# abb128/april-asr

Measured on AMD Instinct MI355X. Metric: audio_seconds_per_second (concurrent 16 kHz sessions x 1/RTF), aprilv0_en-us-sized streaming RNN-T, higher is better.
Workload: dtype f32

## Files before the change

april_asr_amd/csrc/kernels_gemm_kw.hip:

```cpp
#include "kernels.h"
#include "device_utils.h"
#include <algorithm>
#include <atomic>
#include <cstdio>
#include <cstdlib>

namespace aprilx {

namespace {

template <class T> __device__ __forceinline__ T gload(const void *p) { return *(const __attribute__((address_space(1))) T *)(p); }
template <class T> __device__ __forceinline__ void gstore(void *p, const T &v) { *(__attribute__((address_space(1))) T *)(p) = v; }

template <int N> __device__ __forceinline__ void wait_vm()
{
    __builtin_amdgcn_s_waitcnt(0x0F70 | (N & 15) | ((N >> 4) << 14));
}
__device__ __forceinline__ void wait_lgkm0() { __builtin_amdgcn_s_waitcnt(0xC07F); }

constexpr int NW = 8, D = 2;
template <int MT, int NT> struct KwGeom {
    static constexpr int BM = 16 * MT, BN = 16 * NT, LDR = BN + 4, NTH = 64 * NW;
    static constexpr int STAGE_BYTES = BM * 128;
    static constexpr int RING_BYTES = D * STAGE_BYTES, PLANE_BYTES = BM * LDR * 4;
    static constexpr int WAVE_BYTES = ((RING_BYTES > PLANE_BYTES ? RING_BYTES : PLANE_BYTES) + 1023) / 1024 * 1024;
    static constexpr int LDS_MAIN = NW * WAVE_BYTES;
    static constexpr int PLANE = WAVE_BYTES / 4;
    static constexpr int NPIECE = 2 * MT;
    static constexpr int LX = NPIECE, LY = 2 * NT, GSZ = LX + LY;
};

template <int MT, int NT, int EPI, int CPW>
__device__ __forceinline__ void gemm_kw_body(const GemmArgs &g, const int bx, const int by, const unsigned wg_linear)
{
    using G = KwGeom<MT, NT>;
    constexpr int BM = G::BM, BN = G::BN, LDR = G::LDR, NTH = G::NTH, PLANE = G::PLANE;
    constexpr bool ROW_EPI = EPI == EPI_HR || EPI == EPI_RESID_SSQ;
    static_assert(ROW_EPI, "no GM_KW form of this epilogue");
    static_assert(CPW == 1 || CPW == 4, "a wave owns one chunk or one slab");
    constexpr bool DB1 = MT * NT >= 16;
    extern __shared__ __attribute__((aligned(1024))) float red[];
    char *lds = reinterpret_cast<char *>(red);

    if (g.run_flag && gload<int>(g.run_flag) != g.run_gen) return;
    const int lane = threadIdx.x & 63;
    const int wave = __builtin_amdgcn_readfirstlane(threadIdx.x >> 6);
#ifdef APRIL_GEMM_TRACE
    auto stamp = [&](int i) { if (g.trace && wave == 0) g.trace[(size_t)wg_linear * 16 + i] = __builtin_amdgcn_s_memtime(); };
    unsigned long long ph_acc[5] = {0, 0, 0, 0, 0}, ph_t = 0;
    auto lap = [&](int i) { const unsigned long long now = __builtin_amdgcn_s_memtime(); ph_acc[i] += now - ph_t; ph_t = now; };
#else
    auto stamp = [](int) {};
    auto lap = [](int) {};
    (void)wg_linear;
#endif
    stamp(0);
    const int nt0 = bx * NT, n0 = bx * BN, m0 = by * BM;
    const int KB = g.K >> 4;
    const int c = KB / (4 * g.kz);
    constexpr int cpw = CPW;
    const int T = cpw * c;
// ... 30 lines not shown
        }
        if (aidx) {
#pragma unroll
            for (int i = 0; i < G::NPIECE; ++i) arows[i] = gload<int>(aidx + arows[i]);
        }
#pragma unroll
        for (int i = 0; i < G::NPIECE; ++i) {
            const int R = i * 8 + (lane >> 3);
            const int gseg = (lane & 7) ^ ((R >> 1) & 7);
            aoff[i] = (uint32_t)((size_t)arows[i] * lda * 4 + gseg * 16);
        }
    }
    char *my = lds + wave * G::WAVE_BYTES;
    auto issue_dma = [&](int slot) {
#ifdef APRIL_KW_ABLATE
        if (g.debug == 4 || g.debug == 6 || g.debug == 7 || g.debug == 9) return;
#endif
#pragma unroll
        for (int i = 0; i < G::NPIECE; ++i) {
            __builtin_amdgcn_global_load_lds((const __attribute__((address_space(1))) void *)(abase + aoff[i]),
                                             (__attribute__((address_space(3))) void *)(my + slot * G::STAGE_BYTES + i * 1024), 16, 0, 0);
        }
#ifdef APRIL_KW_ABLATE
        if (g.debug == 3) return;
#endif
        abase += 128;
    };
    const char *bp = reinterpret_cast<const char *>(g.wp) + ((size_t)nt0 * KB + first_kb) * 1024;
    const size_t bstride = (size_t)KB * 1024;
    const uint32_t boff = (uint32_t)lane * 16u;
    constexpr int DB = DB1 ? 1 : D;
    f32x4 be[DB][NT], bo[DB][NT];
#ifdef APRIL_KW_ABLATE
#pragma unroll
    for (int t = 0; t < DB; ++t)
#pragma unroll
        for (int nt = 0; nt < NT; ++nt) { be[t][nt] = f32x4{1.f, 1.f, 1.f, 1.f}; bo[t][nt] = be[t][nt]; }
#endif
    auto load_b = [&](f32x4 (&b)[NT]) {
#ifdef APRIL_KW_ABLATE
        if (g.debug == 6 || g.debug == 7 || g.debug == 8) {
#pragma unroll
            for (int nt = 0; nt < NT; ++nt) asm volatile("" : "+v"(b[nt]));
            return;
        }
#endif
#pragma unroll
        for (int nt = 0; nt < NT; ++nt) b[nt] = gload<f32x4>(bp + nt * bstride + boff);
#ifdef APRIL_KW_ABLATE
        if (g.debug == 3) return;
#endif
        bp += 1024;
    };

    constexpr int QROW = BN / 4, NQ = BM * QROW, QPT = (NQ + NTH - 1) / NTH;
    f32x4 e_bias[QPT], e_res[QPT];
// ... 9 lines not shown
        const int qn = q < NQ ? n0 + (q % QROW) * 4 : n0;
        e_bias[i] = (EPI != EPI_HR) ? gload<f32x4>(g.bias + qn) : f32x4{0.f, 0.f, 0.f, 0.f};
        e_slot[i] = (EPI == EPI_HR && g.slot_idx) ? gload<int>(g.slot_idx + m) : m;
        e_res[i] = (EPI == EPI_HR || (EPI == EPI_RESID_SSQ && g.resid)) ? gload<f32x4>(g.resid + (size_t)m * g.ldr + qn) : f32x4{0.f, 0.f, 0.f, 0.f};
    }
    };
    constexpr bool LATE_EPI = DB1 || (MT == 1 && EPI == EPI_HR);
    if constexpr (!LATE_EPI) fetch_epilogue_operands();

    const int mrow = lane & 15, kq = lane >> 4;
    int a_rd[2];
#pragma unroll
    for (int p = 0; p < 2; ++p) a_rd[p] = mrow * 128 + (((p * 4 + kq) ^ ((mrow >> 1) & 7)) << 4);
    auto read_frags = [&](int slot, int p, f32x4 (&a)[MT]) {
#ifdef APRIL_KW_ABLATE
        if (g.debug == 6) {
#pragma unroll
            for (int mt = 0; mt < MT; ++mt) asm volatile("" : "+v"(a[mt]));
            return;
        }
#endif
#pragma unroll
        for (int mt = 0; mt < MT; ++mt) a[mt] = *reinterpret_cast<const f32x4 *>(my + slot * G::STAGE_BYTES + a_rd[p] + mt * 2048);
    };

    f32x4 acc[MT][NT], S[CPW == 4 ? MT : 1][CPW == 4 ? NT : 1];
#define APRIL_KW_EACH(expr) _Pragma("unroll") for (int mt = 0; mt < MT; ++mt) _Pragma("unroll") for (int nt = 0; nt < NT; ++nt) { expr; }
    APRIL_KW_EACH(acc[mt][nt] = (f32x4{0.f, 0.f, 0.f, 0.f}))
    int chunk_i = 0, in_chunk = 0;
    auto fold = [&]() {
        if constexpr (CPW == 4) {
            const bool first = chunk_i == 0;
#pragma unroll
            for (int mt = 0; mt < MT; ++mt)
#pragma unroll
                for (int nt = 0; nt < NT; ++nt) {
                    S[mt][nt] = first ? acc[mt][nt] : S[mt][nt] + acc[mt][nt];
                    acc[mt][nt] = f32x4{0.f, 0.f, 0.f, 0.f};
                    if constexpr (MT * NT >= 16) __builtin_amdgcn_sched_barrier(0);
                }
            ++chunk_i;
        }
    };
    auto mfma_block = [&](const f32x4 (&a)[MT], const f32x4 (&b)[NT]) {
#ifdef APRIL_KW_ABLATE
// ... 45 lines not shown
                    __builtin_amdgcn_sched_barrier(0);
                }
                wait_lgkm0();
                if (more_a) issue_dma(slot);
                if (more_b) load_b(be[0]);
#pragma unroll
                for (int mt = 0; mt < MT; ++mt) {
                    mfma_mt(mt, bo[0]);
                    __builtin_amdgcn_sched_barrier(0);
                    if (mt == 0) { if (more_a) wait_vm<G::NPIECE + 3 * NT>(); else if (more_b) wait_vm<3 * NT>(); }
                    read_frag1(slot ^ 1, 0, mt);
                    __builtin_amdgcn_sched_barrier(0);
                }
                if (more_b) load_b(bo[0]);
                if constexpr (CPW == 4) { if (++in_chunk == cs) { in_chunk = 0; fold(); } }
            }
        }
    } else
    if (g.debug != 1) {
#pragma unroll
        for (int t = 0; t < D; ++t) { issue_dma(t); load_b(be[t]); load_b(bo[t]); }
        wait_vm<(D - 1) * G::GSZ + G::LY>();
        __builtin_amdgcn_sched_barrier(0);
        read_frags(0, 0, a0);
        stamp(1);
        auto stage = [&](const int slot, const bool more, auto wait_next) {
            read_frags(slot, 1, a1);
            __builtin_amdgcn_sched_barrier(0);
            mfma_block(a0, be[slot]);
            __builtin_amdgcn_sched_barrier(0);
// ... 80 lines not shown
        } else {
            const bool ok = e_ok[i];
            f32x4 y = f32x4{0.f, 0.f, 0.f, 0.f};
            if (ok) {
                y = resid_tail(v, e_bias[i], e_res[i], g.resid != nullptr);
                gstore<f32x4>(g.out + (size_t)m * g.ldo + n, y);
            }
            float ss;
            if (granule_ssq_store(y, ok, q, ss)) gstore<float>(g.ssq_out + (size_t)m * (g.N / SSQ_COLS) + n / SSQ_COLS, ss);
        }
    }
    stamp(4);
#undef APRIL_KW_EACH
}

template <int MT, int NT, int EPI, int CPW>
__global__ __launch_bounds__(64 * NW, (MT == 1 && EPI == EPI_HR) ? 6 : 2) void gemm_kw_kernel(GemmArgs g)
{
    gemm_kw_body<MT, NT, EPI, CPW>(g, (int)blockIdx.x, (int)blockIdx.y, blockIdx.x + gridDim.x * blockIdx.y);
}

template <int MT, int NT, int EPI, int CPW>
__global__ __launch_bounds__(64 * NW, (MT == 1 && EPI == EPI_HR) ? 6 : 2) void gemm_kw_zkernel(const GemmArgs *__restrict__ zargs)
{
    const GemmArgs g = zargs[blockIdx.z];
    gemm_kw_body<MT, NT, EPI, CPW>(g, (int)blockIdx.x, (int)blockIdx.y, blockIdx.x + gridDim.x * (blockIdx.y + gridDim.y * blockIdx.z));
}

template <int MT, int NT, int EPI, int CPW>
void launch_kw_one(const GemmArgs &g, const GemmArgs *dev_args, int n, hipStream_t s)
{
    using G = KwGeom<MT, NT>;
    dim3 grid((unsigned)(g.N / G::BN), (unsigned)((g.M + G::BM - 1) / G::BM), (unsigned)std::max(1, n));
    const size_t lds = (size_t)G::LDS_MAIN + scale_lds_floats(g, G::BM) * sizeof(float);
    launch_gemm_pair<&gemm_kw_kernel<MT, NT, EPI, CPW>, &gemm_kw_zkernel<MT, NT, EPI, CPW>>(grid, dim3(G::NTH), lds, true, s, g, dev_args);
}

template <int MT, int NT>
bool dispatch_kw(const GemmArgs &g, const GemmArgs *dev_args, int n, hipStream_t s)
{
    const int cpw = 4 * g.kz / NW;
    if (g.epi == EPI_HR && cpw == 4) { launch_kw_one<MT, NT, EPI_HR, 4>(g, dev_args, n, s); return true; }
    if (g.epi == EPI_HR && cpw == 1) { launch_kw_one<MT, NT, EPI_HR, 1>(g, dev_args, n, s); return true; }
    if (g.epi == EPI_RESID_SSQ && cpw == 4) { launch_kw_one<MT, NT, EPI_RESID_SSQ, 4>(g, dev_args, n, s); return true; }
    if (g.epi == EPI_RESID_SSQ && cpw == 1) { launch_kw_one<MT, NT, EPI_RESID_SSQ, 1>(g, dev_args, n, s); return true; }
    return false;
}

}

// ... 28 lines not shown
```

Measured before the change: 20490.

## Add hand-scheduled inline-asm main loop for split-K GEMM tiles

Replaces the compiler-generated K loop of the wave-split-K GEMM, for the NT=2, MT=1 or 2, four-chunks-per-wave forms, with a hand-written inline-assembly loop. The loop interleaves MFMA instructions with LDS DMA issues, B-operand global loads and LDS fragment reads, and uses explicit waitcnt values and an in-register chunk fold. The aim is tighter overlap of memory traffic with matrix math and fewer compiler-inserted stalls. In exchange it hardcodes register allocation and wait counts, adds a large fragile asm block, and can be turned off with an environment variable.

```diff
diff --git a/april_asr_amd/csrc/gemm_kw_asm.inc b/april_asr_amd/csrc/gemm_kw_asm.inc
--- /dev/null
+++ b/april_asr_amd/csrc/gemm_kw_asm.inc
@@ -0,0 +1,693 @@
+#define APRIL_KWLOOP_M2_TEXT \
+    "s_mov_b32 s90, m0\n" \
+    "s_mov_b64 s[80:81], %[ap]\n" \
+    "s_mov_b64 s[82:83], %[bp0]\n" \
+    "s_mov_b64 s[84:85], %[bp1]\n" \
+    "s_mov_b32 s89, %[lds]\n" \
+    "s_lshr_b32 s86, %[nst], 1\n" \
+    "s_sub_u32 s86, s86, 1\n" \
+    "s_mov_b32 s88, %[cs]\n" \
+    "s_mov_b32 s87, 0\n" \
+    "s_nop 4\n" \
+    "s_add_u32 m0, s89, 0\n" \
+    "s_nop 0\n" \
+    "global_load_lds_dwordx4 %[ao0], s[80:81]\n" \
+    "s_add_u32 m0, s89, 1024\n" \
+    "s_nop 0\n" \
+    "global_load_lds_dwordx4 %[ao1], s[80:81]\n" \
+    "s_add_u32 m0, s89, 2048\n" \
+    "s_nop 0\n" \
+    "global_load_lds_dwordx4 %[ao2], s[80:81]\n" \
+    "s_add_u32 m0, s89, 3072\n" \
+    "s_nop 0\n" \
+    "global_load_lds_dwordx4 %[ao3], s[80:81]\n" \
+    "s_add_u32 s80, s80, 128\n" \
+    "s_addc_u32 s81, s81, 0\n" \
+    "global_load_dwordx4 v[88:91], %[bo], s[82:83]\n" \
+    "global_load_dwordx4 v[92:95], %[bo], s[84:85]\n" \
+    "global_load_dwordx4 v[96:99], %[bo], s[82:83] offset:1024\n" \
+    "global_load_dwordx4 v[100:103], %[bo], s[84:85] offset:1024\n" \
+    "s_add_u32 s82, s82, 2048\n" \
+    "s_addc_u32 s83, s83, 0\n" \
+    "s_add_u32 s84, s84, 2048\n" \
+    "s_addc_u32 s85, s85, 0\n" \
+    "s_add_u32 m0, s89, 4096\n" \
+    "s_nop 0\n" \
+    "global_load_lds_dwordx4 %[ao0], s[80:81]\n" \
+    "s_add_u32 m0, s89, 5120\n" \
+    "s_nop 0\n" \
+    "global_load_lds_dwordx4 %[ao1], s[80:81]\n" \
+    "s_add_u32 m0, s89, 6144\n" \
+    "s_nop 0\n" \
+    "global_load_lds_dwordx4 %[ao2], s[80:81]\n" \
+    "s_add_u32 m0, s89, 7168\n" \
+    "s_nop 0\n" \
+    "global_load_lds_dwordx4 %[ao3], s[80:81]\n" \
+    "s_add_u32 s80, s80, 128\n" \
+    "s_addc_u32 s81, s81, 0\n" \
+    "global_load_dwordx4 v[104:107], %[bo], s[82:83]\n" \
+    "global_load_dwordx4 v[108:111], %[bo], s[84:85]\n" \
+    "global_load_dwordx4 v[112:115], %[bo], s[82:83] offset:1024\n" \
+    "global_load_dwordx4 v[116:119], %[bo], s[84:85] offset:1024\n" \
+    "s_add_u32 s82, s82, 2048\n" \
+    "s_addc_u32 s83, s83, 0\n" \
+    "s_add_u32 s84, s84, 2048\n" \
+    "s_addc_u32 s85, s85, 0\n" \
+    "v_bfrev_b32 v40, 1\n" \
+    "v_bfrev_b32 v41, 1\n" \
+    "v_bfrev_b32 v42, 1\n" \
+    "v_bfrev_b32 v43, 1\n" \
+    "v_bfrev_b32 v56, 1\n" \
+    "v_bfrev_b32 v57, 1\n" \
+    "v_bfrev_b32 v58, 1\n" \
+    "v_bfrev_b32 v59, 1\n" \
+    "v_bfrev_b32 v44, 1\n" \
+    "v_bfrev_b32 v45, 1\n" \
+    "v_bfrev_b32 v46, 1\n" \
+    "v_bfrev_b32 v47, 1\n" \
+    "v_bfrev_b32 v60, 1\n" \
+    "v_bfrev_b32 v61, 1\n" \
+    "v_bfrev_b32 v62, 1\n" \
+    "v_bfrev_b32 v63, 1\n" \
+    "v_bfrev_b32 v48, 1\n" \
+    "v_bfrev_b32 v49, 1\n" \
+    "v_bfrev_b32 v50, 1\n" \
+    "v_bfrev_b32 v51, 1\n" \
+    "v_bfrev_b32 v64, 1\n" \
+    "v_bfrev_b32 v65, 1\n" \
+    "v_bfrev_b32 v66, 1\n" \
+    "v_bfrev_b32 v67, 1\n" \
+    "v_bfrev_b32 v52, 1\n" \
+    "v_bfrev_b32 v53, 1\n" \
+    "v_bfrev_b32 v54, 1\n" \
+    "v_bfrev_b32 v55, 1\n" \
+    "v_bfrev_b32 v68, 1\n" \
+    "v_bfrev_b32 v69, 1\n" \
+    "v_bfrev_b32 v70, 1\n" \
+    "v_bfrev_b32 v71, 1\n" \
+    "s_waitcnt vmcnt(12)\n" \
+    "ds_read_b128 v[72:75], %[rd0] offset:0\n" \
+    "ds_read_b128 v[76:79], %[rd0] offset:2048\n" \
+    "s_waitcnt lgkmcnt(0)\n" \
+    "s_cmp_eq_u32 s86, 0\n" \
+    "s_cbranch_scc1 L_tail_%=\n" \
+    "L_top_%=:\n" \
+    "s_waitcnt vmcnt(10)\n" \
+    "s_cmp_eq_u32 s87, 0\n" \
+    "s_cbranch_scc0 L_nfb0_%=\n" \
+    "v_add_f32 v40, v40, v56\n" \
+    "v_add_f32 v41, v41, v57\n" \
+    "v_add_f32 v42, v42, v58\n" \
+    "v_add_f32 v43, v43, v59\n" \
+    "v_mfma_f32_16x16x4_f32 v[56:59], v72, v88, 0\n" \
+    "v_add_f32 v44, v44, v60\n" \
+    "v_add_f32 v45, v45, v61\n" \
+    "v_add_f32 v46, v46, v62\n" \
+    "v_add_f32 v47, v47, v63\n" \
+    "v_mfma_f32_16x16x4_f32 v[60:63], v72, v92, 0\n" \
+    "v_add_f32 v48, v48, v64\n" \
+    "v_add_f32 v49, v49, v65\n" \
+    "v_add_f32 v50, v50, v66\n" \
+    "v_add_f32 v51, v51, v67\n" \
+    "v_mfma_f32_16x16x4_f32 v[64:67], v76, v88, 0\n" \
+    "v_add_f32 v52, v52, v68\n" \
+    "v_add_f32 v53, v53, v69\n" \
+    "v_add_f32 v54, v54, v70\n" \
+    "v_add_f32 v55, v55, v71\n" \
+    "v_mfma_f32_16x16x4_f32 v[68:71], v76, v92, 0\n" \
+    "s_mov_b32 s87, s88\n" \
+    "s_branch L_jb0_%=\n" \
+    "L_nfb0_%=:\n" \
+    "v_mfma_f32_16x16x4_f32 v[56:59], v72, v88, v[56:59]\n" \
+    "v_mfma_f32_16x16x4_f32 v[60:63], v72, v92, v[60:63]\n" \
+    "v_mfma_f32_16x16x4_f32 v[64:67], v76, v88, v[64:67]\n" \
+    "v_mfma_f32_16x16x4_f32 v[68:71], v76, v92, v[68:71]\n" \
+    "L_jb0_%=:\n" \
+    "v_mfma_f32_16x16x4_f32 v[56:59], v73, v89, v[56:59]\n" \
+    "s_sub_u32 s87, s87, 1\n" \
+    "ds_read_b128 v[80:83], %[rd1] offset:0\n" \
+    "v_mfma_f32_16x16x4_f32 v[60:63], v73, v93, v[60:63]\n" \
+    "ds_read_b128 v[84:87], %[rd1] offset:2048\n" \
+    "v_mfma_f32_16x16x4_f32 v[64:67], v77, v89, v[64:67]\n" \
+    "v_mfma_f32_16x16x4_f32 v[68:71], v77, v93, v[68:71]\n" \
+    "v_mfma_f32_16x16x4_f32 v[56:59], v74, v90, v[56:59]\n" \
+    "s_waitcnt lgkmcnt(0)\n" \
+    "s_add_u32 m0, s89, 0\n" \
+    "v_mfma_f32_16x16x4_f32 v[60:63], v74, v94, v[60:63]\n" \
+    "global_load_lds_dwordx4 %[ao0], s[80:81]\n" \
+    "s_add_u32 m0, s89, 1024\n" \
+    "v_mfma_f32_16x16x4_f32 v[64:67], v78, v90, v[64:67]\n" \
+    "global_load_lds_dwordx4 %[ao1], s[80:81]\n" \
+    "s_add_u32 m0, s89, 2048\n" \
+    "v_mfma_f32_16x16x4_f32 v[68:71], v78, v94, v[68:71]\n" \
+    "global_load_lds_dwordx4 %[ao2], s[80:81]\n" \
+    "s_add_u32 m0, s89, 3072\n" \
+    "v_mfma_f32_16x16x4_f32 v[56:59], v75, v91, v[56:59]\n" \
+    "global_load_lds_dwordx4 %[ao3], s[80:81]\n" \
+    "s_add_u32 s80, s80, 128\n" \
+    "s_addc_u32 s81, s81, 0\n" \
+    "v_mfma_f32_16x16x4_f32 v[60:63], v75, v95, v[60:63]\n" \
+    "v_mfma_f32_16x16x4_f32 v[64:67], v79, v91, v[64:67]\n" \
+    "v_mfma_f32_16x16x4_f32 v[68:71], v79, v95, v[68:71]\n" \
+    "s_waitcnt vmcnt(8)\n" \
+    "ds_read_b128 v[72:75], %[rd0] offset:4096\n" \
+    "v_mfma_f32_16x16x4_f32 v[56:59], v80, v96, v[56:59]\n" \
+    "ds_read_b128 v[76:79], %[rd0] offset:6144\n" \
+    "v_mfma_f32_16x16x4_f32 v[60:63], v80, v100, v[60:63]\n" \
+    "v_mfma_f32_16x16x4_f32 v[64:67], v84, v96, v[64:67]\n" \
+    "global_load_dwordx4 v[88:91], %[bo], s[82:83]\n" \
+    "v_mfma_f32_16x16x4_f32 v[68:71], v84, v100, v[68:71]\n" \
+    "v_mfma_f32_16x16x4_f32 v[56:59], v81, v97, v[56:59]\n" \
+    "global_load_dwordx4 v[92:95], %[bo], s[84:85]\n" \
+    "v_mfma_f32_16x16x4_f32 v[60:63], v81, v101, v[60:63]\n" \
+    "v_mfma_f32_16x16x4_f32 v[64:67], v85, v97, v[64:67]\n" \
+    "v_mfma_f32_16x16x4_f32 v[68:71], v85, v101, v[68:71]\n" \
+    "v_mfma_f32_16x16x4_f32 v[56:59], v82, v98, v[56:59]\n" \
+    "v_mfma_f32_16x16x4_f32 v[60:63], v82, v102, v[60:63]\n" \
+    "v_mfma_f32_16x16x4_f32 v[64:67], v86, v98, v[64:67]\n" \
+    "v_mfma_f32_16x16x4_f32 v[68:71], v86, v102, v[68:71]\n" \
+    "v_mfma_f32_16x16x4_f32 v[56:59], v83, v99, v[56:59]\n" \
+    "v_mfma_f32_16x16x4_f32 v[60:63], v83, v103, v[60:63]\n" \
+    "v_mfma_f32_16x16x4_f32 v[64:67], v87, v99, v[64:67]\n" \
+    "global_load_dwordx4 v[96:99], %[bo], s[82:83] offset:1024\n" \
+    "v_mfma_f32_16x16x4_f32 v[68:71], v87, v103, v[68:71]\n" \
+    "global_load_dwordx4 v[100:103], %[bo], s[84:85] offset:1024\n" \
+    "s_add_u32 s82, s82, 2048\n" \
+    "s_addc_u32 s83, s83, 0\n" \
+    "s_add_u32 s84, s84, 2048\n" \
+    "s_addc_u32 s85, s85, 0\n" \
+    "s_waitcnt lgkmcnt(0)\n" \
+    "s_waitcnt vmcnt(10)\n" \
+    "s_cmp_eq_u32 s87, 0\n" \
+    "s_cbranch_scc0 L_nfb1_%=\n" \
+    "v_add_f32 v40, v40, v56\n" \
+    "v_add_f32 v41, v41, v57\n" \
+    "v_add_f32 v42, v42, v58\n" \
+    "v_add_f32 v43, v43, v59\n" \
+    "v_mfma_f32_16x16x4_f32 v[56:59], v72, v104, 0\n" \
+    "v_add_f32 v44, v44, v60\n" \
+    "v_add_f32 v45, v45, v61\n" \
+    "v_add_f32 v46, v46, v62\n" \
+    "v_add_f32 v47, v47, v63\n" \
+    "v_mfma_f32_16x16x4_f32 v[60:63], v72, v108, 0\n" \
+    "v_add_f32 v48, v48, v64\n" \
+    "v_add_f32 v49, v49, v65\n" \
+    "v_add_f32 v50, v50, v66\n" \
+    "v_add_f32 v51, v51, v67\n" \
+    "v_mfma_f32_16x16x4_f32 v[64:67], v76, v104, 0\n" \
+    "v_add_f32 v52, v52, v68\n" \
+    "v_add_f32 v53, v53, v69\n" \
+    "v_add_f32 v54, v54, v70\n" \
+    "v_add_f32 v55, v55, v71\n" \
+    "v_mfma_f32_16x16x4_f32 v[68:71], v76, v108, 0\n" \
+    "s_mov_b32 s87, s88\n" \
+    "s_branch L_jb1_%=\n" \
+    "L_nfb1_%=:\n" \
+    "v_mfma_f32_16x16x4_f32 v[56:59], v72, v104, v[56:59]\n" \
+    "v_mfma_f32_16x16x4_f32 v[60:63], v72, v108, v[60:63]\n" \
+    "v_mfma_f32_16x16x4_f32 v[64:67], v76, v104, v[64:67]\n" \
+    "v_mfma_f32_16x16x4_f32 v[68:71], v76, v108, v[68:71]\n" \
+    "L_jb1_%=:\n" \
+    "v_mfma_f32_16x16x4_f32 v[56:59], v73, v105, v[56:59]\n" \
+    "s_sub_u32 s87, s87, 1\n" \
+    "ds_read_b128 v[80:83], %[rd1] offset:4096\n" \
+    "v_mfma_f32_16x16x4_f32 v[60:63], v73, v109, v[60:63]\n" \
+    "ds_read_b128 v[84:87], %[rd1] offset:6144\n" \
+    "v_mfma_f32_16x16x4_f32 v[64:67], v77, v105, v[64:67]\n" \
+    "v_mfma_f32_16x16x4_f32 v[68:71], v77, v109, v[68:71]\n" \
+    "v_mfma_f32_16x16x4_f32 v[56:59], v74, v106, v[56:59]\n" \
+    "s_waitcnt lgkmcnt(0)\n" \
+    "s_add_u32 m0, s89, 4096\n" \
+    "v_mfma_f32_16x16x4_f32 v[60:63], v74, v110, v[60:63]\n" \
+    "global_load_lds_dwordx4 %[ao0], s[80:81]\n" \
+    "s_add_u32 m0, s89, 5120\n" \
+    "v_mfma_f32_16x16x4_f32 v[64:67], v78, v106, v[64:67]\n" \
+    "global_load_lds_dwordx4 %[ao1], s[80:81]\n" \
+    "s_add_u32 m0, s89, 6144\n" \
+    "v_mfma_f32_16x16x4_f32 v[68:71], v78, v110, v[68:71]\n" \
+    "global_load_lds_dwordx4 %[ao2], s[80:81]\n" \
+    "s_add_u32 m0, s89, 7168\n" \
+    "v_mfma_f32_16x16x4_f32 v[56:59], v75, v107, v[56:59]\n" \
+    "global_load_lds_dwordx4 %[ao3], s[80:81]\n" \
+    "s_add_u32 s80, s80, 128\n" \
+    "s_addc_u32 s81, s81, 0\n" \
+    "v_mfma_f32_16x16x4_f32 v[60:63], v75, v111, v[60:63]\n" \
+    "v_mfma_f32_16x16x4_f32 v[64:67], v79, v107, v[64:67]\n" \
+    "v_mfma_f32_16x16x4_f32 v[68:71], v79, v111, v[68:71]\n" \
+    "s_waitcnt vmcnt(8)\n" \
+    "ds_read_b128 v[72:75], %[rd0] offset:0\n" \
+    "v_mfma_f32_16x16x4_f32 v[56:59], v80, v112, v[56:59]\n" \
+    "ds_read_b128 v[76:79], %[rd0] offset:2048\n" \
+    "v_mfma_f32_16x16x4_f32 v[60:63], v80, v116, v[60:63]\n" \
+    "v_mfma_f32_16x16x4_f32 v[64:67], v84, v112, v[64:67]\n" \
+    "global_load_dwordx4 v[104:107], %[bo], s[82:83]\n" \
+    "v_mfma_f32_16x16x4_f32 v[68:71], v84, v116, v[68:71]\n" \
+    "v_mfma_f32_16x16x4_f32 v[56:59], v81, v113, v[56:59]\n" \
+    "global_load_dwordx4 v[108:111], %[bo], s[84:85]\n" \
+    "v_mfma_f32_16x16x4_f32 v[60:63], v81, v117, v[60:63]\n" \
+    "v_mfma_f32_16x16x4_f32 v[64:67], v85, v113, v[64:67]\n" \
+    "v_mfma_f32_16x16x4_f32 v[68:71], v85, v117, v[68:71]\n" \
+    "v_mfma_f32_16x16x4_f32 v[56:59], v82, v114, v[56:59]\n" \
+    "v_mfma_f32_16x16x4_f32 v[60:63], v82, v118, v[60:63]\n" \
+    "v_mfma_f32_16x16x4_f32 v[64:67], v86, v114, v[64:67]\n" \
+    "v_mfma_f32_16x16x4_f32 v[68:71], v86, v118, v[68:71]\n" \
+    "v_mfma_f32_16x16x4_f32 v[56:59], v83, v115, v[56:59]\n" \
+    "v_mfma_f32_16x16x4_f32 v[60:63], v83, v119, v[60:63]\n" \
+    "v_mfma_f32_16x16x4_f32 v[64:67], v87, v115, v[64:67]\n" \
+    "global_load_dwordx4 v[112:115], %[bo], s[82:83] offset:1024\n" \
+    "v_mfma_f32_16x16x4_f32 v[68:71], v87, v119, v[68:71]\n" \
+    "global_load_dwordx4 v[116:119], %[bo], s[84:85] offset:1024\n" \
+    "s_add_u32 s82, s82, 2048\n" \
+    "s_addc_u32 s83, s83, 0\n" \
+    "s_add_u32 s84, s84, 2048\n" \
+    "s_addc_u32 s85, s85, 0\n" \
+    "s_waitcnt lgkmcnt(0)\n" \
+    "s_sub_u32 s86, s86, 1\n" \
+    "s_cmp_lg_u32 s86, 0\n" \
+    "s_cbranch_scc1 L_top_%=\n" \
+    "L_tail_%=:\n" \
+    "s_waitcnt vmcnt(10)\n" \
+    "s_cmp_eq_u32 s87, 0\n" \
+    "s_cbranch_scc0 L_nft0_%=\n" \
+    "v_add_f32 v40, v40, v56\n" \
+    "v_add_f32 v41, v41, v57\n" \
+    "v_add_f32 v42, v42, v58\n" \
+    "v_add_f32 v43, v43, v59\n" \
+    "v_mfma_f32_16x16x4_f32 v[56:59], v72, v88, 0\n" \
+    "v_add_f32 v44, v44, v60\n" \
+    "v_add_f32 v45, v45, v61\n" \
+    "v_add_f32 v46, v46, v62\n" \
+    "v_add_f32 v47, v47, v63\n" \
+    "v_mfma_f32_16x16x4_f32 v[60:63], v72, v92, 0\n" \
+    "v_add_f32 v48, v48, v64\n" \
+    "v_add_f32 v49, v49, v65\n" \
+    "v_add_f32 v50, v50, v66\n" \
+    "v_add_f32 v51, v51, v67\n" \
+    "v_mfma_f32_16x16x4_f32 v[64:67], v76, v88, 0\n" \
+    "v_add_f32 v52, v52, v68\n" \
+    "v_add_f32 v53, v53, v69\n" \
+    "v_add_f32 v54, v54, v70\n" \
+    "v_add_f32 v55, v55, v71\n" \
+    "v_mfma_f32_16x16x4_f32 v[68:71], v76, v92, 0\n" \
+    "s_mov_b32 s87, s88\n" \
+    "s_branch L_jt0_%=\n" \
+    "L_nft0_%=:\n" \
+    "v_mfma_f32_16x16x4_f32 v[56:59], v72, v88, v[56:59]\n" \
+    "v_mfma_f32_16x16x4_f32 v[60:63], v72, v92, v[60:63]\n" \
+    "v_mfma_f32_16x16x4_f32 v[64:67], v76, v88, v[64:67]\n" \
+    "v_mfma_f32_16x16x4_f32 v[68:71], v76, v92, v[68:71]\n" \
+    "L_jt0_%=:\n" \
+    "v_mfma_f32_16x16x4_f32 v[56:59], v73, v89, v[56:59]\n" \
+    "s_sub_u32 s87, s87, 1\n" \
+    "ds_read_b128 v[80:83], %[rd1] offset:0\n" \
+    "v_mfma_f32_16x16x4_f32 v[60:63], v73, v93, v[60:63]\n" \
+    "ds_read_b128 v[84:87], %[rd1] offset:2048\n" \
+    "v_mfma_f32_16x16x4_f32 v[64:67], v77, v89, v[64:67]\n" \
+    "v_mfma_f32_16x16x4_f32 v[68:71], v77, v93, v[68:71]\n" \
+    "v_mfma_f32_16x16x4_f32 v[56:59], v74, v90, v[56:59]\n" \
+    "s_waitcnt lgkmcnt(0)\n" \
+    "v_mfma_f32_16x16x4_f32 v[60:63], v74, v94, v[60:63]\n" \
+    "v_mfma_f32_16x16x4_f32 v[64:67], v78, v90, v[64:67]\n" \
+    "v_mfma_f32_16x16x4_f32 v[68:71], v78, v94, v[68:71]\n" \
+    "v_mfma_f32_16x16x4_f32 v[56:59], v75, v91, v[56:59]\n" \
+    "v_mfma_f32_16x16x4_f32 v[60:63], v75, v95, v[60:63]\n" \
+    "v_mfma_f32_16x16x4_f32 v[64:67], v79, v91, v[64:67]\n" \
+    "v_mfma_f32_16x16x4_f32 v[68:71], v79, v95, v[68:71]\n" \
+    "s_waitcnt vmcnt(4)\n" \
+    "ds_read_b128 v[72:75], %[rd0] offset:4096\n" \
+    "v_mfma_f32_16x16x4_f32 v[56:59], v80, v96, v[56:59]\n" \
+    "ds_read_b128 v[76:79], %[rd0] offset:6144\n" \
+    "v_mfma_f32_16x16x4_f32 v[60:63], v80, v100, v[60:63]\n" \
+    "v_mfma_f32_16x16x4_f32 v[64:67], v84, v96, v[64:67]\n" \
+    "v_mfma_f32_16x16x4_f32 v[68:71], v84, v100, v[68:71]\n" \
+    "v_mfma_f32_16x16x4_f32 v[56:59], v81, v97, v[56:59]\n" \
+    "v_mfma_f32_16x16x4_f32 v[60:63], v81, v101, v[60:63]\n" \
+    "v_mfma_f32_16x16x4_f32 v[64:67], v85, v97, v[64:67]\n" \
+    "v_mfma_f32_16x16x4_f32 v[68:71], v85, v101, v[68:71]\n" \
+    "v_mfma_f32_16x16x4_f32 v[56:59], v82, v98, v[56:59]\n" \
+    "v_mfma_f32_16x16x4_f32 v[60:63], v82, v102, v[60:63]\n" \
+    "v_mfma_f32_16x16x4_f32 v[64:67], v86, v98, v[64:67]\n" \
+    "v_mfma_f32_16x16x4_f32 v[68:71], v86, v102, v[68:71]\n" \
+    "v_mfma_f32_16x16x4_f32 v[56:59], v83, v99, v[56:59]\n" \
+    "v_mfma_f32_16x16x4_f32 v[60:63], v83, v103, v[60:63]\n" \
+    "v_mfma_f32_16x16x4_f32 v[64:67], v87, v99, v[64:67]\n" \
+    "v_mfma_f32_16x16x4_f32 v[68:71], v87, v103, v[68:71]\n" \
+    "s_waitcnt lgkmcnt(0)\n" \
+    "s_waitcnt vmcnt(2)\n" \
+    "s_cmp_eq_u32 s87, 0\n" \
+    "s_cbranch_scc0 L_nft1_%=\n" \
+    "v_add_f32 v40, v40, v56\n" \
+    "v_add_f32 v41, v41, v57\n" \
+    "v_add_f32 v42, v42, v58\n" \
+    "v_add_f32 v43, v43, v59\n" \
+    "v_mfma_f32_16x16x4_f32 v[56:59], v72, v104, 0\n" \
+    "v_add_f32 v44, v44, v60\n" \
+    "v_add_f32 v45, v45, v61\n" \
+    "v_add_f32 v46, v46, v62\n" \
+    "v_add_f32 v47, v47, v63\n" \
+    "v_mfma_f32_16x16x4_f32 v[60:63], v72, v108, 0\n" \
+    "v_add_f32 v48, v48, v64\n" \
+    "v_add_f32 v49, v49, v65\n" \
+    "v_add_f32 v50, v50, v66\n" \
+    "v_add_f32 v51, v51, v67\n" \
+    "v_mfma_f32_16x16x4_f32 v[64:67], v76, v104, 0\n" \
+    "v_add_f32 v52, v52, v68\n" \
+    "v_add_f32 v53, v53, v69\n" \
+    "v_add_f32 v54, v54, v70\n" \
+    "v_add_f32 v55, v55, v71\n" \
+    "v_mfma_f32_16x16x4_f32 v[68:71], v76, v108, 0\n" \
+    "s_mov_b32 s87, s88\n" \
+    "s_branch L_jt1_%=\n" \
+    "L_nft1_%=:\n" \
+    "v_mfma_f32_16x16x4_f32 v[56:59], v72, v104, v[56:59]\n" \
+    "v_mfma_f32_16x16x4_f32 v[60:63], v72, v108, v[60:63]\n" \
+    "v_mfma_f32_16x16x4_f32 v[64:67], v76, v104, v[64:67]\n" \
+    "v_mfma_f32_16x16x4_f32 v[68:71], v76, v108, v[68:71]\n" \
+    "L_jt1_%=:\n" \
+    "v_mfma_f32_16x16x4_f32 v[56:59], v73, v105, v[56:59]\n" \
+    "s_sub_u32 s87, s87, 1\n" \
+    "ds_read_b128 v[80:83], %[rd1] offset:4096\n" \
+    "v_mfma_f32_16x16x4_f32 v[60:63], v73, v109, v[60:63]\n" \
+    "ds_read_b128 v[84:87], %[rd1] offset:6144\n" \
+    "v_mfma_f32_16x16x4_f32 v[64:67], v77, v105, v[64:67]\n" \
+    "v_mfma_f32_16x16x4_f32 v[68:71], v77, v109, v[68:71]\n" \
+    "v_mfma_f32_16x16x4_f32 v[56:59], v74, v106, v[56:59]\n" \
+    "s_waitcnt lgkmcnt(0)\n" \
+    "v_mfma_f32_16x16x4_f32 v[60:63], v74, v110, v[60:63]\n" \
+    "v_mfma_f32_16x16x4_f32 v[64:67], v78, v106, v[64:67]\n" \
+    "v_mfma_f32_16x16x4_f32 v[68:71], v78, v110, v[68:71]\n" \
+    "v_mfma_f32_16x16x4_f32 v[56:59], v75, v107, v[56:59]\n" \
+    "v_mfma_f32_16x16x4_f32 v[60:63], v75, v111, v[60:63]\n" \
+    "v_mfma_f32_16x16x4_f32 v[64:67], v79, v107, v[64:67]\n" \
+    "v_mfma_f32_16x16x4_f32 v[68:71], v79, v111, v[68:71]\n" \
+    "s_waitcnt vmcnt(0)\n" \
+    "v_mfma_f32_16x16x4_f32 v[56:59], v80, v112, v[56:59]\n" \
+    "v_mfma_f32_16x16x4_f32 v[60:63], v80, v116, v[60:63]\n" \
+    "v_mfma_f32_16x16x4_f32 v[64:67], v84, v112, v[64:67]\n" \
+    "v_mfma_f32_16x16x4_f32 v[68:71], v84, v116, v[68:71]\n" \
+    "v_mfma_f32_16x16x4_f32 v[56:59], v81, v113, v[56:59]\n" \
+    "v_mfma_f32_16x16x4_f32 v[60:63], v81, v117, v[60:63]\n" \
+    "v_mfma_f32_16x16x4_f32 v[64:67], v85, v113, v[64:67]\n" \
+    "v_mfma_f32_16x16x4_f32 v[68:71], v85, v117, v[68:71]\n" \
+    "v_mfma_f32_16x16x4_f32 v[56:59], v82, v114, v[56:59]\n" \
+    "v_mfma_f32_16x16x4_f32 v[60:63], v82, v118, v[60:63]\n" \
+    "v_mfma_f32_16x16x4_f32 v[64:67], v86, v114, v[64:67]\n" \
+    "v_mfma_f32_16x16x4_f32 v[68:71], v86, v118, v[68:71]\n" \
+    "v_mfma_f32_16x16x4_f32 v[56:59], v83, v115, v[56:59]\n" \
+    "v_mfma_f32_16x16x4_f32 v[60:63], v83, v119, v[60:63]\n" \
+    "v_mfma_f32_16x16x4_f32 v[64:67], v87, v115, v[64:67]\n" \
+    "v_mfma_f32_16x16x4_f32 v[68:71], v87, v119, v[68:71]\n" \
+    "s_nop 7\n" \
+    "s_nop 7\n" \
+    "v_add_f32 v40, v40, v56\n" \
+    "v_add_f32 v41, v41, v57\n" \
+    "v_add_f32 v42, v42, v58\n" \
+    "v_add_f32 v43, v43, v59\n" \
+    "v_add_f32 v44, v44, v60\n" \
+    "v_add_f32 v45, v45, v61\n" \
+    "v_add_f32 v46, v46, v62\n" \
+    "v_add_f32 v47, v47, v63\n" \
+    "v_add_f32 v48, v48, v64\n" \
+    "v_add_f32 v49, v49, v65\n" \
+    "v_add_f32 v50, v50, v66\n" \
+    "v_add_f32 v51, v51, v67\n" \
+    "v_add_f32 v52, v52, v68\n" \
+    "v_add_f32 v53, v53, v69\n" \
+    "v_add_f32 v54, v54, v70\n" \
+    "v_add_f32 v55, v55, v71\n" \
+    "s_mov_b32 m0, s90\n"
+#define APRIL_KWLOOP_M2_CLOBBERS "v56", "v57", "v58", "v59", "v60", "v61", "v62", "v63", "v64", "v65", "v66", "v67", "v68", "v69", "v70", "v71", "v72", "v73", "v74", "v75", "v76", "v77", "v78", "v79", "v80", "v81", "v82", "v83", "v84", "v85", "v86", "v87", "v88", "v89", "v90", "v91", "v92", "v93", "v94", "v95", "v96", "v97", "v98", "v99", "v100", "v101", "v102", "v103", "v104", "v105", "v106", "v107", "v108", "v109", "v110", "v111", "v112", "v113", "v114", "v115", "v116", "v117", "v118", "v119", "s80", "s81", "s82", "s83", "s84", "s85", "s86", "s87", "s88", "s89", "s90", "scc", "memory"
+#define APRIL_KWLOOP_M2_S0 "=&{v[40:43]}"
+#define APRIL_KWLOOP_M2_S1 "=&{v[44:47]}"
+#define APRIL_KWLOOP_M2_S2 "=&{v[48:51]}"
+#define APRIL_KWLOOP_M2_S3 "=&{v[52:55]}"
+
+#define APRIL_KWLOOP_M1_TEXT \
+    "s_mov_b32 s90, m0\n" \
+    "s_mov_b64 s[80:81], %[ap]\n" \
+    "s_mov_b64 s[82:83], %[bp0]\n" \
+    "s_mov_b64 s[84:85], %[bp1]\n" \
+    "s_mov_b32 s89, %[lds]\n" \
+    "s_lshr_b32 s86, %[nst], 1\n" \
+    "s_sub_u32 s86, s86, 1\n" \
+    "s_mov_b32 s88, %[cs]\n" \
+    "s_mov_b32 s87, 0\n" \
+    "s_nop 4\n" \
+    "s_add_u32 m0, s89, 0\n" \
+    "s_nop 0\n" \
+    "global_load_lds_dwordx4 %[ao0], s[80:81]\n" \
+    "s_add_u32 m0, s89, 1024\n" \
+    "s_nop 0\n" \
+    "global_load_lds_dwordx4 %[ao1], s[80:81]\n" \
+    "s_add_u32 s80, s80, 128\n" \
+    "s_addc_u32 s81, s81, 0\n" \
+    "global_load_dwordx4 v[48:51], %[bo], s[82:83]\n" \
+    "global_load_dwordx4 v[52:55], %[bo], s[84:85]\n" \
+    "global_load_dwordx4 v[56:59], %[bo], s[82:83] offset:1024\n" \
+    "global_load_dwordx4 v[60:63], %[bo], s[84:85] offset:1024\n" \
+    "s_add_u32 s82, s82, 2048\n" \
+    "s_addc_u32 s83, s83, 0\n" \
+    "s_add_u32 s84, s84, 2048\n" \
+    "s_addc_u32 s85, s85, 0\n" \
+    "s_add_u32 m0, s89, 2048\n" \
+    "s_nop 0\n" \
+    "global_load_lds_dwordx4 %[ao0], s[80:81]\n" \
+    "s_add_u32 m0, s89, 3072\n" \
+    "s_nop 0\n" \
+    "global_load_lds_dwordx4 %[ao1], s[80:81]\n" \
+    "s_add_u32 s80, s80, 128\n" \
+    "s_addc_u32 s81, s81, 0\n" \
+    "global_load_dwordx4 v[64:67], %[bo], s[82:83]\n" \
+    "global_load_dwordx4 v[68:71], %[bo], s[84:85]\n" \
+    "global_load_dwordx4 v[72:75], %[bo], s[82:83] offset:1024\n" \
+    "global_load_dwordx4 v[76:79], %[bo], s[84:85] offset:1024\n" \
+    "s_add_u32 s82, s82, 2048\n" \
+    "s_addc_u32 s83, s83, 0\n" \
+    "s_add_u32 s84, s84, 2048\n" \
+    "s_addc_u32 s85, s85, 0\n" \
+    "v_bfrev_b32 v24, 1\n" \
+    "v_bfrev_b32 v25, 1\n" \
+    "v_bfrev_b32 v26, 1\n" \
+    "v_bfrev_b32 v27, 1\n" \
+    "v_bfrev_b32 v32, 1\n" \
+    "v_bfrev_b32 v33, 1\n" \
+    "v_bfrev_b32 v34, 1\n" \
+    "v_bfrev_b32 v35, 1\n" \
+    "v_bfrev_b32 v28, 1\n" \
+    "v_bfrev_b32 v29, 1\n" \
+    "v_bfrev_b32 v30, 1\n" \
+    "v_bfrev_b32 v31, 1\n" \
+    "v_bfrev_b32 v36, 1\n" \
+    "v_bfrev_b32 v37, 1\n" \
+    "v_bfrev_b32 v38, 1\n" \
+    "v_bfrev_b32 v39, 1\n" \
+    "s_waitcnt vmcnt(10)\n" \
+    "ds_read_b128 v[40:43], %[rd0] offset:0\n" \
+    "s_waitcnt lgkmcnt(0)\n" \
+    "s_cmp_eq_u32 s86, 0\n" \
+    "s_cbranch_scc1 L_tail_%=\n" \
+    "L_top_%=:\n" \
+    "s_waitcnt vmcnt(8)\n" \
+    "s_cmp_eq_u32 s87, 0\n" \
+    "s_cbranch_scc0 L_nfb0_%=\n" \
+    "s_nop 7\n" \
+    "v_add_f32 v24, v24, v32\n" \
+    "v_add_f32 v25, v25, v33\n" \
+    "v_add_f32 v26, v26, v34\n" \
+    "v_add_f32 v27, v27, v35\n" \
+    "v_mfma_f32_16x16x4_f32 v[32:35], v40, v48, 0\n" \
+    "v_add_f32 v28, v28, v36\n" \
+    "v_add_f32 v29, v29, v37\n" \
+    "v_add_f32 v30, v30, v38\n" \
+    "v_add_f32 v31, v31, v39\n" \
+    "v_mfma_f32_16x16x4_f32 v[36:39], v40, v52, 0\n" \
+    "s_mov_b32 s87, s88\n" \
+    "s_branch L_jb0_%=\n" \
+    "L_nfb0_%=:\n" \
+    "v_mfma_f32_16x16x4_f32 v[32:35], v40, v48, v[32:35]\n" \
+    "v_mfma_f32_16x16x4_f32 v[36:39], v40, v52, v[36:39]\n" \
+    "L_jb0_%=:\n" \
+    "v_mfma_f32_16x16x4_f32 v[32:35], v41, v49, v[32:35]\n" \
+    "s_sub_u32 s87, s87, 1\n" \
+    "ds_read_b128 v[44:47], %[rd1] offset:0\n" \
+    "v_mfma_f32_16x16x4_f32 v[36:39], v41, v53, v[36:39]\n" \
+    "v_mfma_f32_16x16x4_f32 v[32:35], v42, v50, v[32:35]\n" \
+    "s_waitcnt lgkmcnt(0)\n" \
+    "s_add_u32 m0, s89, 0\n" \
+    "v_mfma_f32_16x16x4_f32 v[36:39], v42, v54, v[36:39]\n" \
+    "global_load_lds_dwordx4 %[ao0], s[80:81]\n" \
+    "s_add_u32 m0, s89, 1024\n" \
+    "v_mfma_f32_16x16x4_f32 v[32:35], v43, v51, v[32:35]\n" \
+    "global_load_lds_dwordx4 %[ao1], s[80:81]\n" \
+    "s_add_u32 s80, s80, 128\n" \
+    "s_addc_u32 s81, s81, 0\n" \
+    "v_mfma_f32_16x16x4_f32 v[36:39], v43, v55, v[36:39]\n" \
+    "s_waitcnt vmcnt(6)\n" \
+    "ds_read_b128 v[40:43], %[rd0] offset:2048\n" \
+    "v_mfma_f32_16x16x4_f32 v[32:35], v44, v56, v[32:35]\n" \
+    "v_mfma_f32_16x16x4_f32 v[36:39], v44, v60, v[36:39]\n" \
+    "v_mfma_f32_16x16x4_f32 v[32:35], v45, v57, v[32:35]\n" \
+    "global_load_dwordx4 v[48:51], %[bo], s[82:83]\n" \
+    "v_mfma_f32_16x16x4_f32 v[36:39], v45, v61, v[36:39]\n" \
+    "v_mfma_f32_16x16x4_f32 v[32:35], v46, v58, v[32:35]\n" \
+    "global_load_dwordx4 v[52:55], %[bo], s[84:85]\n" \
+    "v_mfma_f32_16x16x4_f32 v[36:39], v46, v62, v[36:39]\n" \
+    "v_mfma_f32_16x16x4_f32 v[32:35], v47, v59, v[32:35]\n" \
+    "global_load_dwordx4 v[56:59], %[bo], s[82:83] offset:1024\n" \
+    "v_mfma_f32_16x16x4_f32 v[36:39], v47, v63, v[36:39]\n" \
+    "global_load_dwordx4 v[60:63], %[bo], s[84:85] offset:1024\n" \
+    "s_add_u32 s82, s82, 2048\n" \
+    "s_addc_u32 s83, s83, 0\n" \
+    "s_add_u32 s84, s84, 2048\n" \
+    "s_addc_u32 s85, s85, 0\n" \
+    "s_waitcnt lgkmcnt(0)\n" \
+    "s_waitcnt vmcnt(8)\n" \
+    "s_cmp_eq_u32 s87, 0\n" \
+    "s_cbranch_scc0 L_nfb1_%=\n" \
+    "s_nop 7\n" \
+    "v_add_f32 v24, v24, v32\n" \
+    "v_add_f32 v25, v25, v33\n" \
+    "v_add_f32 v26, v26, v34\n" \
+    "v_add_f32 v27, v27, v35\n" \
+    "v_mfma_f32_16x16x4_f32 v[32:35], v40, v64, 0\n" \
+    "v_add_f32 v28, v28, v36\n" \
+    "v_add_f32 v29, v29, v37\n" \
+    "v_add_f32 v30, v30, v38\n" \
+    "v_add_f32 v31, v31, v39\n" \
+    "v_mfma_f32_16x16x4_f32 v[36:39], v40, v68, 0\n" \
+    "s_mov_b32 s87, s88\n" \
+    "s_branch L_jb1_%=\n" \
+    "L_nfb1_%=:\n" \
+    "v_mfma_f32_16x16x4_f32 v[32:35], v40, v64, v[32:35]\n" \
+    "v_mfma_f32_16x16x4_f32 v[36:39], v40, v68, v[36:39]\n" \
+    "L_jb1_%=:\n" \
+    "v_mfma_f32_16x16x4_f32 v[32:35], v41, v65, v[32:35]\n" \
+    "s_sub_u32 s87, s87, 1\n" \
+    "ds_read_b128 v[44:47], %[rd1] offset:2048\n" \
+    "v_mfma_f32_16x16x4_f32 v[36:39], v41, v69, v[36:39]\n" \
+    "v_mfma_f32_16x16x4_f32 v[32:35], v42, v66, v[32:35]\n" \
+    "s_waitcnt lgkmcnt(0)\n" \
+    "s_add_u32 m0, s89, 2048\n" \
+    "v_mfma_f32_16x16x4_f32 v[36:39], v42, v70, v[36:39]\n" \
+    "global_load_lds_dwordx4 %[ao0], s[80:81]\n" \
+    "s_add_u32 m0, s89, 3072\n" \
+    "v_mfma_f32_16x16x4_f32 v[32:35], v43, v67, v[32:35]\n" \
+    "global_load_lds_dwordx4 %[ao1], s[80:81]\n" \
+    "s_add_u32 s80, s80, 128\n" \
+    "s_addc_u32 s81, s81, 0\n" \
+    "v_mfma_f32_16x16x4_f32 v[36:39], v43, v71, v[36:39]\n" \
+    "s_waitcnt vmcnt(6)\n" \
+    "ds_read_b128 v[40:43], %[rd0] offset:0\n" \
+    "v_mfma_f32_16x16x4_f32 v[32:35], v44, v72, v[32:35]\n" \
+    "v_mfma_f32_16x16x4_f32 v[36:39], v44, v76, v[36:39]\n" \
+    "v_mfma_f32_16x16x4_f32 v[32:35], v45, v73, v[32:35]\n" \
+    "global_load_dwordx4 v[64:67], %[bo], s[82:83]\n" \
+    "v_mfma_f32_16x16x4_f32 v[36:39], v45, v77, v[36:39]\n" \
+    "v_mfma_f32_16x16x4_f32 v[32:35], v46, v74, v[32:35]\n" \
+    "global_load_dwordx4 v[68:71], %[bo], s[84:85]\n" \
+    "v_mfma_f32_16x16x4_f32 v[36:39], v46, v78, v[36:39]\n" \
+    "v_mfma_f32_16x16x4_f32 v[32:35], v47, v75, v[32:35]\n" \
+    "global_load_dwordx4 v[72:75], %[bo], s[82:83] offset:1024\n" \
+    "v_mfma_f32_16x16x4_f32 v[36:39], v47, v79, v[36:39]\n" \
+    "global_load_dwordx4 v[76:79], %[bo], s[84:85] offset:1024\n" \
+    "s_add_u32 s82, s82, 2048\n" \
+    "s_addc_u32 s83, s83, 0\n" \
+    "s_add_u32 s84, s84, 2048\n" \
+    "s_addc_u32 s85, s85, 0\n" \
+    "s_waitcnt lgkmcnt(0)\n" \
+    "s_sub_u32 s86, s86, 1\n" \
+    "s_cmp_lg_u32 s86, 0\n" \
+    "s_cbranch_scc1 L_top_%=\n" \
+    "L_tail_%=:\n" \
+    "s_waitcnt vmcnt(8)\n" \
+    "s_cmp_eq_u32 s87, 0\n" \
+    "s_cbranch_scc0 L_nft0_%=\n" \
+    "s_nop 7\n" \
+    "v_add_f32 v24, v24, v32\n" \
+    "v_add_f32 v25, v25, v33\n" \
+    "v_add_f32 v26, v26, v34\n" \
+    "v_add_f32 v27, v27, v35\n" \
+    "v_mfma_f32_16x16x4_f32 v[32:35], v40, v48, 0\n" \
+    "v_add_f32 v28, v28, v36\n" \
+    "v_add_f32 v29, v29, v37\n" \
+    "v_add_f32 v30, v30, v38\n" \
+    "v_add_f32 v31, v31, v39\n" \
+    "v_mfma_f32_16x16x4_f32 v[36:39], v40, v52, 0\n" \
+    "s_mov_b32 s87, s88\n" \
+    "s_branch L_jt0_%=\n" \
+    "L_nft0_%=:\n" \
+    "v_mfma_f32_16x16x4_f32 v[32:35], v40, v48, v[32:35]\n" \
+    "v_mfma_f32_16x16x4_f32 v[36:39], v40, v52, v[36:39]\n" \
+    "L_jt0_%=:\n" \
+    "v_mfma_f32_16x16x4_f32 v[32:35], v41, v49, v[32:35]\n" \
+    "s_sub_u32 s87, s87, 1\n" \
+    "ds_read_b128 v[44:47], %[rd1] offset:0\n" \
+    "v_mfma_f32_16x16x4_f32 v[36:39], v41, v53, v[36:39]\n" \
+    "v_mfma_f32_16x16x4_f32 v[32:35], v42, v50, v[32:35]\n" \
+    "s_waitcnt lgkmcnt(0)\n" \
+    "v_mfma_f32_16x16x4_f32 v[36:39], v42, v54, v[36:39]\n" \
+    "v_mfma_f32_16x16x4_f32 v[32:35], v43, v51, v[32:35]\n" \
+    "v_mfma_f32_16x16x4_f32 v[36:39], v43, v55, v[36:39]\n" \
+    "s_waitcnt vmcnt(4)\n" \
+    "ds_read_b128 v[40:43], %[rd0] offset:2048\n" \
+    "v_mfma_f32_16x16x4_f32 v[32:35], v44, v56, v[32:35]\n" \
+    "v_mfma_f32_16x16x4_f32 v[36:39], v44, v60, v[36:39]\n" \
+    "v_mfma_f32_16x16x4_f32 v[32:35], v45, v57, v[32:35]\n" \
+    "v_mfma_f32_16x16x4_f32 v[36:39], v45, v61, v[36:39]\n" \
+    "v_mfma_f32_16x16x4_f32 v[32:35], v46, v58, v[32:35]\n" \
+    "v_mfma_f32_16x16x4_f32 v[36:39], v46, v62, v[36:39]\n" \
+    "v_mfma_f32_16x16x4_f32 v[32:35], v47, v59, v[32:35]\n" \
+    "v_mfma_f32_16x16x4_f32 v[36:39], v47, v63, v[36:39]\n" \
+    "s_waitcnt lgkmcnt(0)\n" \
+    "s_waitcnt vmcnt(2)\n" \
+    "s_cmp_eq_u32 s87, 0\n" \
+    "s_cbranch_scc0 L_nft1_%=\n" \
+    "s_nop 7\n" \
+    "v_add_f32 v24, v24, v32\n" \
+    "v_add_f32 v25, v25, v33\n" \
+    "v_add_f32 v26, v26, v34\n" \
+    "v_add_f32 v27, v27, v35\n" \
+    "v_mfma_f32_16x16x4_f32 v[32:35], v40, v64, 0\n" \
+    "v_add_f32 v28, v28, v36\n" \
+    "v_add_f32 v29, v29, v37\n" \
+    "v_add_f32 v30, v30, v38\n" \
+    "v_add_f32 v31, v31, v39\n" \
+    "v_mfma_f32_16x16x4_f32 v[36:39], v40, v68, 0\n" \
+    "s_mov_b32 s87, s88\n" \
+    "s_branch L_jt1_%=\n" \
+    "L_nft1_%=:\n" \
+    "v_mfma_f32_16x16x4_f32 v[32:35], v40, v64, v[32:35]\n" \
+    "v_mfma_f32_16x16x4_f32 v[36:39], v40, v68, v[36:39]\n" \
+    "L_jt1_%=:\n" \
+    "v_mfma_f32_16x16x4_f32 v[32:35], v41, v65, v[32:35]\n" \
+    "s_sub_u32 s87, s87, 1\n" \
+    "ds_read_b128 v[44:47], %[rd1] offset:2048\n" \
+    "v_mfma_f32_16x16x4_f32 v[36:39], v41, v69, v[36:39]\n" \
+    "v_mfma_f32_16x16x4_f32 v[32:35], v42, v66, v[32:35]\n" \
+    "s_waitcnt lgkmcnt(0)\n" \
+    "v_mfma_f32_16x16x4_f32 v[36:39], v42, v70, v[36:39]\n" \
+    "v_mfma_f32_16x16x4_f32 v[32:35], v43, v67, v[32:35]\n" \
+    "v_mfma_f32_16x16x4_f32 v[36:39], v43, v71, v[36:39]\n" \
+    "s_waitcnt vmcnt(0)\n" \
+    "v_mfma_f32_16x16x4_f32 v[32:35], v44, v72, v[32:35]\n" \
+    "v_mfma_f32_16x16x4_f32 v[36:39], v44, v76, v[36:39]\n" \
+    "v_mfma_f32_16x16x4_f32 v[32:35], v45, v73, v[32:35]\n" \
+    "v_mfma_f32_16x16x4_f32 v[36:39], v45, v77, v[36:39]\n" \
+    "v_mfma_f32_16x16x4_f32 v[32:35], v46, v74, v[32:35]\n" \
+    "v_mfma_f32_16x16x4_f32 v[36:39], v46, v78, v[36:39]\n" \
+    "v_mfma_f32_16x16x4_f32 v[32:35], v47, v75, v[32:35]\n" \
+    "v_mfma_f32_16x16x4_f32 v[36:39], v47, v79, v[36:39]\n" \
+    "s_nop 7\n" \
+    "s_nop 7\n" \
+    "v_add_f32 v24, v24, v32\n" \
+    "v_add_f32 v25, v25, v33\n" \
+    "v_add_f32 v26, v26, v34\n" \
+    "v_add_f32 v27, v27, v35\n" \
+    "v_add_f32 v28, v28, v36\n" \
+    "v_add_f32 v29, v29, v37\n" \
+    "v_add_f32 v30, v30, v38\n" \
+    "v_add_f32 v31, v31, v39\n" \
+    "s_mov_b32 m0, s90\n"
+#define APRIL_KWLOOP_M1_CLOBBERS "v32", "v33", "v34", "v35", "v36", "v37", "v38", "v39", "v40", "v41", "v42", "v43", "v44", "v45", "v46", "v47", "v48", "v49", "v50", "v51", "v52", "v53", "v54", "v55", "v56", "v57", "v58", "v59", "v60", "v61", "v62", "v63", "v64", "v65", "v66", "v67", "v68", "v69", "v70", "v71", "v72", "v73", "v74", "v75", "v76", "v77", "v78", "v79", "s80", "s81", "s82", "s83", "s84", "s85", "s86", "s87", "s88", "s89", "s90", "scc", "memory"
+#define APRIL_KWLOOP_M1_S0 "=&{v[24:27]}"
+#define APRIL_KWLOOP_M1_S1 "=&{v[28:31]}"
diff --git a/april_asr_amd/csrc/kernels_gemm_kw.hip b/april_asr_amd/csrc/kernels_gemm_kw.hip
--- a/april_asr_amd/csrc/kernels_gemm_kw.hip
+++ b/april_asr_amd/csrc/kernels_gemm_kw.hip
@@ -1,5 +1,7 @@
 #include "kernels.h"
 #include "device_utils.h"
+#include "env.h"
+#include "gemm_kw_asm.inc"
 #include <algorithm>
 #include <atomic>
 #include <cstdio>
@@ -30,7 +32,9 @@
     static constexpr int LX = NPIECE, LY = 2 * NT, GSZ = LX + LY;
 };
 
-template <int MT, int NT, int EPI, int CPW>
+template <int MT, int NT> constexpr bool kw_has_hand(int cpw) { return NT == 2 && (MT == 1 || MT == 2) && cpw == 4; }
+
+template <int MT, int NT, int EPI, int CPW, bool HAND>
 __device__ __forceinline__ void gemm_kw_body(const GemmArgs &g, const int bx, const int by, const unsigned wg_linear)
 {
     using G = KwGeom<MT, NT>;
@@ -38,6 +42,7 @@
     constexpr bool ROW_EPI = EPI == EPI_HR || EPI == EPI_RESID_SSQ;
     static_assert(ROW_EPI, "no GM_KW form of this epilogue");
     static_assert(CPW == 1 || CPW == 4, "a wave owns one chunk or one slab");
+    static_assert(!HAND || kw_has_hand<MT, NT>(CPW), "no hand-placed loop for this form");
     constexpr bool DB1 = MT * NT >= 16;
     extern __shared__ __attribute__((aligned(1024))) float red[];
     char *lds = reinterpret_cast<char *>(red);
@@ -45,6 +50,10 @@
     if (g.run_flag && gload<int>(g.run_flag) != g.run_gen) return;
     const int lane = threadIdx.x & 63;
     const int wave = __builtin_amdgcn_readfirstlane(threadIdx.x >> 6);
+#ifdef APRIL_KW_ABLATE
+    const bool abl_nofold = g.debug == 10 || g.debug == 11;
+    const int abl = g.debug == 10 ? 6 : g.debug == 11 ? 7 : g.debug;
+#endif
 #ifdef APRIL_GEMM_TRACE
     auto stamp = [&](int i) { if (g.trace && wave == 0) g.trace[(size_t)wg_linear * 16 + i] = __builtin_amdgcn_s_memtime(); };
     unsigned long long ph_acc[5] = {0, 0, 0, 0, 0}, ph_t = 0;
@@ -105,7 +114,7 @@
     char *my = lds + wave * G::WAVE_BYTES;
     auto issue_dma = [&](int slot) {
 #ifdef APRIL_KW_ABLATE
-        if (g.debug == 4 || g.debug == 6 || g.debug == 7 || g.debug == 9) return;
+        if (abl == 4 || abl == 6 || abl == 7 || abl == 9) return;
 #endif
 #pragma unroll
         for (int i = 0; i < G::NPIECE; ++i) {
@@ -130,7 +139,7 @@
 #endif
     auto load_b = [&](f32x4 (&b)[NT]) {
 #ifdef APRIL_KW_ABLATE
-        if (g.debug == 6 || g.debug == 7 || g.debug == 8) {
+        if (abl == 6 || abl == 7 || abl == 8) {
 #pragma unroll
             for (int nt = 0; nt < NT; ++nt) asm volatile("" : "+v"(b[nt]));
             return;
@@ -170,7 +179,7 @@
     for (int p = 0; p < 2; ++p) a_rd[p] = mrow * 128 + (((p * 4 + kq) ^ ((mrow >> 1) & 7)) << 4);
     auto read_frags = [&](int slot, int p, f32x4 (&a)[MT]) {
 #ifdef APRIL_KW_ABLATE
-        if (g.debug == 6) {
+        if (abl == 6) {
 #pragma unroll
             for (int mt = 0; mt < MT; ++mt) asm volatile("" : "+v"(a[mt]));
             return;
@@ -185,6 +194,9 @@
     APRIL_KW_EACH(acc[mt][nt] = (f32x4{0.f, 0.f, 0.f, 0.f}))
     int chunk_i = 0, in_chunk = 0;
     auto fold = [&]() {
+#ifdef APRIL_KW_ABLATE
+        if (abl_nofold) return;
+#endif
         if constexpr (CPW == 4) {
             const bool first = chunk_i == 0;
 #pragma unroll
@@ -260,6 +272,26 @@
                 }
                 if (more_b) load_b(bo[0]);
                 if constexpr (CPW == 4) { if (++in_chunk == cs) { in_chunk = 0; fold(); } }
+            }
+        }
+    } else if constexpr (HAND) {
+        if (g.debug != 1) {
+            stamp(1);
+            const uint32_t lds_my = __builtin_amdgcn_readfirstlane((uint32_t)(uintptr_t)(__attribute__((address_space(3))) char *)my);
+            const uint32_t rd0 = lds_my + (uint32_t)a_rd[0], rd1 = lds_my + (uint32_t)a_rd[1];
+            const char *bp1 = bp + bstride;
+            if constexpr (MT == 2) {
+                asm volatile(APRIL_KWLOOP_M2_TEXT
+                             : APRIL_KWLOOP_M2_S0(S[0][0]), APRIL_KWLOOP_M2_S1(S[0][1]), APRIL_KWLOOP_M2_S2(S[1][0]), APRIL_KWLOOP_M2_S3(S[1][1])
+                             : [ao0] "v"(aoff[0]), [ao1] "v"(aoff[1]), [ao2] "v"(aoff[2]), [ao3] "v"(aoff[3]), [bo] "v"(boff), [rd0] "v"(rd0), [rd1] "v"(rd1),
+                               [ap] "s"(abase), [bp0] "s"(bp), [bp1] "s"(bp1), [lds] "s"(lds_my), [nst] "s"(nstage), [cs] "s"(cs)
+                             : APRIL_KWLOOP_M2_CLOBBERS);
+            } else {
+                asm volatile(APRIL_KWLOOP_M1_TEXT
+                             : APRIL_KWLOOP_M1_S0(S[0][0]), APRIL_KWLOOP_M1_S1(S[0][1])
+                             : [ao0] "v"(aoff[0]), [ao1] "v"(aoff[1]), [bo] "v"(boff), [rd0] "v"(rd0), [rd1] "v"(rd1),
+                               [ap] "s"(abase), [bp0] "s"(bp), [bp1] "s"(bp1), [lds] "s"(lds_my), [nst] "s"(nstage), [cs] "s"(cs)
+                             : APRIL_KWLOOP_M1_CLOBBERS);
             }
         }
     } else
@@ -370,26 +402,31 @@
 #undef APRIL_KW_EACH
 }
 
-template <int MT, int NT, int EPI, int CPW>
+template <int MT, int NT, int EPI, int CPW, bool HAND>
 __global__ __launch_bounds__(64 * NW, (MT == 1 && EPI == EPI_HR) ? 6 : 2) void gemm_kw_kernel(GemmArgs g)
 {
-    gemm_kw_body<MT, NT, EPI, CPW>(g, (int)blockIdx.x, (int)blockIdx.y, blockIdx.x + gridDim.x * blockIdx.y);
-}
-
-template <int MT, int NT, int EPI, int CPW>
+    gemm_kw_body<MT, NT, EPI, CPW, HAND>(g, (int)blockIdx.x, (int)blockIdx.y, blockIdx.x + gridDim.x * blockIdx.y);
+}
+
+template <int MT, int NT, int EPI, int CPW, bool HAND>
 __global__ __launch_bounds__(64 * NW, (MT == 1 && EPI == EPI_HR) ? 6 : 2) void gemm_kw_zkernel(const GemmArgs *__restrict__ zargs)
 {
     const GemmArgs g = zargs[blockIdx.z];
-    gemm_kw_body<MT, NT, EPI, CPW>(g, (int)blockIdx.x, (int)blockIdx.y, blockIdx.x + gridDim.x * (blockIdx.y + gridDim.y * blockIdx.z));
+    gemm_kw_body<MT, NT, EPI, CPW, HAND>(g, (int)blockIdx.x, (int)blockIdx.y, blockIdx.x + gridDim.x * (blockIdx.y + gridDim.y * blockIdx.z));
 }
 
 template <int MT, int NT, int EPI, int CPW>
 void launch_kw_one(const GemmArgs &g, const GemmArgs *dev_args, int n, hipStream_t s)
 {
     using G = KwGeom<MT, NT>;
+    static const int hand = env_int("APRIL_KW_ASM", 1);
     dim3 grid((unsigned)(g.N / G::BN), (unsigned)((g.M + G::BM - 1) / G::BM), (unsigned)std::max(1, n));
     const size_t lds = (size_t)G::LDS_MAIN + scale_lds_floats(g, G::BM) * sizeof(float);
-    launch_gemm_pair<&gemm_kw_kernel<MT, NT, EPI, CPW>, &gemm_kw_zkernel<MT, NT, EPI, CPW>>(grid, dim3(G::NTH), lds, true, s, g, dev_args);
+    if constexpr (kw_has_hand<MT, NT>(CPW)) if (hand && g.debug == 0) {
+        launch_gemm_pair<&gemm_kw_kernel<MT, NT, EPI, CPW, true>, &gemm_kw_zkernel<MT, NT, EPI, CPW, true>>(grid, dim3(G::NTH), lds, true, s, g, dev_args);
+        return;
+    }
+    launch_gemm_pair<&gemm_kw_kernel<MT, NT, EPI, CPW, false>, &gemm_kw_zkernel<MT, NT, EPI, CPW, false>>(grid, dim3(G::NTH), lds, true, s, g, dev_args);
 }
 
 template <int MT, int NT>
```

After: 21110, median of 6. 3.0% higher.
